# otaviog/align3d

Hardware: AMD Instinct MI355X
Metric: ICP frame-pairs/sec (640x480, 3-lvl, 15 iters) (higher is better)
Workload: dtype f32; 1 GPU; ms3x15 x 64 pairs/GPU, distinct frames, 640x480, 3 lvl x 15 it, HBM-resident (configs[4] shard); pairs_per_gpu=64, global_pairs=64, levels=3, distinct_frames=True, ranks_in_collective=1, collective=none

## Files before the change

### align3d_amd/_abi.py

```python
import ctypes as C
import os
import threading

import numpy as np

A3D_OK = 0
A3D_INVALID_PARAMETER = 1
A3D_MISSING_FIELD = 2
A3D_SOLVE_FAILED = 3
A3D_HIP_ERROR = 4
A3D_NAN_IN_INPUT = 5
A3D_CAST_OVERFLOW = 6

STATUS_NAMES = {
    0: "A3D_OK",
    1: "A3D_INVALID_PARAMETER",
    2: "A3D_MISSING_FIELD",
    3: "A3D_SOLVE_FAILED",
    4: "A3D_HIP_ERROR",
    5: "A3D_NAN_IN_INPUT",
    6: "A3D_CAST_OVERFLOW",
}


# ... 289 lines not shown
    "a3d_pcl_icp_batch_align_device": (_ST, [_P, C.POINTER(PointCloudViewC), C.POINTER(PoseC), C.POINTER(C.c_int32)]),
    "a3d_pcl_icp_batch_results": (_ST, [_P, C.POINTER(PoseC), C.POINTER(C.c_int32)]),
    "a3d_pcl_icp_batch_last_device_ms": (_ST, [_P, C.POINTER(C.c_float)]),
    "a3d_pcl_icp_batch_free": (_ST, [_P]),
    "a3d_bilateral_default_sigmas": (None, [C.POINTER(C.c_double), C.POINTER(C.c_double)]),
    "a3d_bilateral_filter_u16": (
        _ST,
        [_P, _P, C.c_uint64, C.c_uint64, C.c_double, C.c_double, _P, C.POINTER(C.c_uint64)],
    ),
    "a3d_bilateral_filter_u16_device": (_ST, [_P, _P, C.c_uint64, C.c_uint64, C.c_uint64, C.c_double, C.c_double, _P]),
}

DIAG_SIGNATURES = {
    "a3d_image_icp_accumulate_exact": (
        _ST,
        [_P, C.POINTER(IcpParamsC), _P, _P, C.POINTER(PoseC), C.POINTER(GnStateC), C.POINTER(GnStateC)],
    ),
    "a3d_image_icp_accumulate_weighted": (
        _ST,
        [_P, C.POINTER(IcpParamsC), _P, _P, C.POINTER(PoseC), C.POINTER(GnStateC)],
    ),
    "a3d_range_image_download_depth16": (_ST, [_P, _P, C.POINTER(C.c_float), C.POINTER(C.c_int32)]),
    "a3d_backproject_proven": (_ST, [C.c_uint32, C.c_uint32, C.POINTER(C.c_float), C.POINTER(C.c_int32)]),
    "a3d_acos_gate_threshold": (_ST, [C.c_float, C.c_int32, C.POINTER(C.c_float)]),
}

_CSRC = os.path.join(os.path.dirname(os.path.abspath(__file__)), "csrc")
LIB_PATH = os.environ.get("A3D_LIBRARY") or os.path.join(_CSRC, "libalign3d_hip.so")
DIAG_LIB_PATH = os.path.join(_CSRC, "libalign3d_hip_diag.so")
_libs = {}


def load_library(path=None):
    path = os.path.abspath(path or LIB_PATH)
    if path in _libs:
        return _libs[path]
    if not os.path.exists(path):
        raise RuntimeError(
            f"{path} not found: build the HIP extension first "
            "(python -c 'import __graft_entry__ as g; g.build()' or make -C align3d_amd/csrc all)"
        )
    lib = C.CDLL(path)
    for name, (restype, argtypes) in SIGNATURES.items():
        fn = getattr(lib, name)
        fn.restype = restype
        fn.argtypes = argtypes
# ... 32 lines not shown
```

### align3d_amd/csrc/common.hpp

```cpp
#pragma once
#include <hip/hip_runtime.h>

#include <atomic>
#include <memory>
#include <cstdarg>
#include <cstdio>
#include <cstring>
#include <mutex>
#include <string>
#include <utility>
#include <vector>

#include "../../include/align3d_hip.h"
#include "devmath.hpp"

struct a3d_context;

#ifdef A3D_DIAGNOSTICS
#define A3D_DIAG_ENV(name) getenv(name)
#else
#define A3D_DIAG_ENV(name) ((const char*)nullptr)
#endif

namespace a3d {
// ... 78 lines not shown
  hipStream_t copy_stream = nullptr;
  std::vector<hipEvent_t> copy_events;
  unsigned long long grid_capacity = 0;
  struct GridLayoutKey {
    const void* region = nullptr;
    unsigned long long capacity = 0;
    uint32_t cell_bytes = 0, flags_stride = 0, frames = 0, columns = 0;
  } grid_clean;
  uint32_t grid_layout_frames = 0;
  std::vector<std::pair<size_t, uint32_t>> arena_requests;
  struct CachedTable {
    uint32_t key[4];
    void* d;
  };
  std::vector<CachedTable> tables;
  int stream_priority = 0;
  std::mutex stream_mutex;
  std::vector<hipStream_t> side_streams;
  uint64_t build_stats[4] = {0, 0, 0, 0};
  bool build_profiling = false;
  std::vector<hipEvent_t> build_events;
  float last_build_kernel_ms = 0.f;
  uint32_t tiles_per_pair = 0;
  int live_arenas = 0;
  bool zombie = false;
};

namespace a3d {
a3d_status ctx_side_stream(a3d_context* ctx, uint32_t index, hipStream_t* out);
a3d_status ctx_scratch(a3d_context* ctx, int which, size_t bytes, void** out);
a3d_status ctx_block_alloc(a3d_context* ctx, size_t bytes, void** out, size_t* out_bytes);
void ctx_block_release(a3d_context* ctx, void* p, size_t bytes);

struct DeviceArena {
  void* base = nullptr;
  size_t bytes = 0;
  bool slab_slice = false;
  std::atomic<int> refs{0};
  std::mutex fence_mutex;
  std::vector<std::shared_ptr<struct UseFence>> fences;
  std::shared_ptr<struct UseFence> self_fence;
};

struct UseFence {
  std::mutex m;
  hipEvent_t ev = nullptr;
// ... 91 lines not shown
```

### align3d_amd/csrc/devmath.hpp

```cpp
#pragma once
#include <hip/hip_runtime.h>
#include <math.h>

#include <algorithm>
#include <cmath>
#include <stdint.h>

#define A3D_HD __host__ __device__ __forceinline__

namespace a3d {

struct V3 {
  float x, y, z;
};
A3D_HD V3 operator+(V3 a, V3 b) { return {a.x + b.x, a.y + b.y, a.z + b.z}; }
A3D_HD V3 operator-(V3 a, V3 b) { return {a.x - b.x, a.y - b.y, a.z - b.z}; }
A3D_HD V3 operator*(V3 a, float s) { return {a.x * s, a.y * s, a.z * s}; }
A3D_HD V3 operator/(V3 a, float s) { return {a.x / s, a.y / s, a.z / s}; }
A3D_HD float dot(V3 a, V3 b) { return (a.x * b.x + a.y * b.y) + a.z * b.z; }
A3D_HD float norm_squared(V3 a) { return dot(a, a); }
A3D_HD V3 cross(V3 a, V3 b) {
  return {a.y * b.z - a.z * b.y, a.z * b.x - a.x * b.z, a.x * b.y - a.y * b.x};
}

struct Quat {
  float i, j, k, w;
};
struct Pose {
// ... 166 lines not shown

__device__ __forceinline__ V3 backproject_px(uint32_t d, int row, int col, float fx, float fy, float cx, float cy, float scale,
                                             const DivBy dfx, const DivBy dfy, bool focal_ok) {
  V3 p{0.f, 0.f, 0.f};
  if (d > 0) {
    p.z = (float)d * scale;
    const float ax = ((float)col - cx) * p.z, ay = ((float)row - cy) * p.z;
    const bool fast = focal_ok & div_num_ok(ax) & div_num_ok(ay);
    if (__builtin_expect(__builtin_amdgcn_ballot_w64(!fast) != 0ull, 0)) {
      p.x = ax / fx, p.y = ay / fy;
    } else {
      p.x = ax == 0.0f ? ax : div_by(ax, dfx), p.y = ay == 0.0f ? ay : div_by(ay, dfy);
    }
  }
  return p;
}

__device__ __forceinline__ V3 backproject_px_proven(uint32_t d, int row, int col, float cx, float cy, float scale,
                                                    const DivBy dfx, const DivBy dfy) {
  V3 p;
  p.z = (float)d * scale;
  const float ax = ((float)col - cx) * p.z, ay = ((float)row - cy) * p.z;
  p.x = div_by(ax, dfx), p.y = div_by(ay, dfy);
  return p;
}
#endif

inline bool backproject_proven(uint32_t w, uint32_t h, float fx, float fy, float cx, float cy, float scale) {
  if (w == 0 || h == 0 || w > (1u << 24) || h > (1u << 24)) return false;
  if (!(scale >= 1.17549435e-38f)) return false;
  const float zmin = 1.0f * scale, zmax = 65535.0f * scale;
  if (!(zmax <= 3.40282347e38f)) return false;
  auto den_ok = [](float f) { return (std::fabs(f) > 1e-9f) & (std::fabs(f) < 1e9f); };
  auto axis_ok = [&](uint32_t n, float f, float c) {
    if (!den_ok(f) || !std::isfinite(c)) return false;
    float amax = 0.0f, amin = INFINITY;
    bool zero = false;
    const double fl = std::floor(std::min(std::max((double)c, -2.0), (double)n + 1.0));
    const double ks[6] = {0.0, (double)(n - 1), fl - 1.0, fl, fl + 1.0, fl + 2.0};
    for (double kd : ks) {
      const float k = (float)std::min(std::max(kd, 0.0), (double)(n - 1));
      const float a = k - c;
      if (a == 0.0f) {
        if (k != c) return false;
        zero = true;
      } else {
        amax = std::max(amax, std::fabs(a)), amin = std::min(amin, std::fabs(a));
      }
    }
    const float big = amax * zmax;
    if (!(big < 1e9f)) return false;
    if (amin != INFINITY && !(amin * zmin > 1e-20f)) return false;
    return !zero || f > 0.0f;
  };
  return axis_ok(w, fx, cx) && axis_ok(h, fy, cy);
}

#if defined(__HIPCC__)


__device__ __forceinline__ V3 normal_from_neighbours_dev(V3 center, V3 left, V3 right, V3 top, V3 bottom) {
  const float ld = norm_squared(left - center), rd = norm_squared(right - center);
  V3 left_to_right;
  if ((ld < 4.0f * rd) & (4.0f * ld > rd))
    left_to_right = right - left;
  else if (ld < rd)
    left_to_right = center - left;
  else
    left_to_right = right - center;
  const float bd = norm_squared(bottom - center), td = norm_squared(top - center);
  V3 bottom_to_top;
  if ((bd < 4.0f * td) & (4.0f * bd > td))
    bottom_to_top = top - bottom;
  else if (bd < td)
    bottom_to_top = center - bottom;
  else
    bottom_to_top = top - center;
  const V3 n = cross(left_to_right, bottom_to_top);
  const float mag = sqrtf(norm_squared(n));
  V3 out{0.f, 0.f, 0.f};
// ... 42 lines not shown
```

### align3d_amd/csrc/frame.hip

```cpp
#include <cmath>
#include <cstdlib>
#include <memory>

#include "pyramid_ops.hpp"

using namespace a3d;

namespace {

#ifndef A3D_MAX_BATCH
#define A3D_MAX_BATCH 48
#endif
#ifndef A3D_GRID_BUDGET_GB
#define A3D_GRID_BUDGET_GB 4
#endif
constexpr uint32_t MAX_BATCH = A3D_MAX_BATCH;
struct FrameBases {
  char* arena[MAX_BATCH];
};

struct LevelLayout {
  uint32_t w, h;
  size_t points, mask, normals, colors, intensities, imap;
  size_t depth16;
// ... 840 lines not shown
}

#ifdef A3D_DIAGNOSTICS
a3d_status a3d_range_image_download_depth16(a3d_device_image* im, uint16_t* out_depth, float out_backproject[5],
                                            int32_t* out_points_from_depth) {
  A3D_REQUIRE(im && out_depth && out_backproject && out_points_from_depth, A3D_INVALID_PARAMETER, "null argument");
  A3D_REQUIRE(im->depth16, A3D_MISSING_FIELD, "image has no depth plane");
  hipSetDevice(im->ctx->device);
  const size_t n = (size_t)im->width * im->height;
  A3D_HIP_TRY(hipMemcpyAsync(out_depth, im->depth16, n * 2, hipMemcpyDeviceToHost, im->ctx->stream));
  A3D_HIP_TRY(hipStreamSynchronize(im->ctx->stream));
  out_backproject[0] = im->bp_fx, out_backproject[1] = im->bp_fy, out_backproject[2] = im->bp_cx;
  out_backproject[3] = im->bp_cy, out_backproject[4] = im->depth_scale;
  *out_points_from_depth = im->points_from_depth ? 1 : 0;
  return A3D_OK;
}

a3d_status a3d_backproject_proven(uint32_t width, uint32_t height, const float backproject[5], int32_t* out_proven) {
  A3D_REQUIRE(backproject && out_proven, A3D_INVALID_PARAMETER, "null argument");
  const float* k = backproject;
  *out_proven = a3d::backproject_proven(width, height, k[0], k[1], k[2], k[3], k[4]) ? 1 : 0;
  return A3D_OK;
}
#endif

}
```

### align3d_amd/csrc/image_icp.hip

```cpp
#include <cstdlib>
#include <memory>

#include "icp_engine.hpp"

using namespace a3d;

namespace {

struct LevelDesc {
  const float* src_points;
  const uint8_t* src_mask;
  const uint8_t* src_intensities;
  const float* tgt_points;
  const float* tgt_normals;
  const uint8_t* tgt_mask;
  const float* imap;
  uint32_t src_n;
  uint32_t tw, th;
  float fx, fy, cx, cy;
  uint32_t flags;
  uint32_t ppt;
  uint32_t src_w;
  const uint16_t* src_depth;
  const uint16_t* tgt_depth;
  float src_bp[5], tgt_bp[5];
  float src_inv_w;
  uint32_t pad;
};
static_assert(sizeof(LevelDesc) == 160, "LevelDesc layout");

struct Gates {
  float max_distance_sqr;
  float max_color_distance_sqr;
  float dot_reject_max;
};

__device__ __forceinline__ uint32_t f32_as_usize(float x) {
  uint32_t r;
  asm("v_cvt_u32_f32_e32 %0, %1" : "=v"(r) : "v"(x));
  return r;
}
__device__ __forceinline__ int32_t f32_as_i32(float x) {
  int32_t r;
  asm("v_cvt_i32_f32_e32 %0, %1" : "=v"(r) : "v"(x));
  return r;
}

typedef const char __attribute__((address_space(1)))* gptr_c;
template <typename T>
__device__ __forceinline__ T ld(const void* base, uint32_t byte_off) {
  return *(const T __attribute__((address_space(1)))*)((gptr_c)base + byte_off);
}
// ... 9 lines not shown
}


__device__ __forceinline__ uint32_t texel_offset(uint32_t row, uint32_t width, uint32_t col) {
  return (__umul24(row, width) + col) * 4u;
}

__device__ __forceinline__ float bilerp(float v00, float v10, float v01, float v11, float uf, float vf) {
  float u0 = v00 * (1.0f - uf) + v10 * uf;
  float u1 = v01 * (1.0f - uf) + v11 * uf;
  return u0 * (1.0f - vf) + u1 * vf;
}
__device__ __forceinline__ float bilinear_at(const float* imap, uint32_t mw, float u, float v) {
  const uint32_t ui = f32_as_usize(u), vi = f32_as_usize(v);
  const uint32_t o = texel_offset(vi, mw, ui);
  const f32x2 a = ld<f32x2_u>(imap, o), b = ld<f32x2_u>(imap, o + mw * 4u);
  return bilerp(a.x, a.y, b.x, b.y, u - (float)ui, v - (float)vi);
}

struct SrcPx {
  V3 sp;
  uint8_t intensity;
  bool live;
  uint32_t depth, row, col;
};
struct BackProj {
  float fx, fy, cx, cy, scale;
  DivBy dfx, dfy;
};
struct BackProj2 {
  BackProj src, tgt;
};
__device__ __forceinline__ float uniform_f(float x) {
  return __int_as_float(__builtin_amdgcn_readfirstlane(__float_as_int(x)));
}
__device__ __forceinline__ BackProj make_backproj(const float (&k)[5]) {
  BackProj b;
  b.fx = k[0], b.fy = k[1], b.cx = k[2], b.cy = k[3], b.scale = k[4];
  const DivBy dx = div_prepare(b.fx), dy = div_prepare(b.fy);
  b.dfx = DivBy{uniform_f(dx.negz), uniform_f(dx.y)}, b.dfy = DivBy{uniform_f(dy.negz), uniform_f(dy.y)};
  return b;
}
constexpr int D16_TGT = 1, D16_SRC = 2;
#ifndef A3D_ICP_DEPTH16_SRC
#define A3D_ICP_DEPTH16_SRC 1
#endif
constexpr int D16_SIDES = D16_TGT | (A3D_ICP_DEPTH16_SRC ? D16_SRC : 0);
template <bool ZMASK = false, int D16 = 0>
__device__ __forceinline__ SrcPx stage_a(const LevelDesc& d, uint32_t i, bool in_range) {
  const uint32_t ii = in_range ? i : 0u;
  SrcPx s;
  if (D16 & D16_SRC) {
    const uint32_t r = f32_as_usize(((float)ii + 0.5f) * d.src_inv_w);
    s.row = r, s.col = ii - __umul24(r, d.src_w);
    s.depth = ld<uint16_t>(d.src_depth, ii * 2u);
    s.intensity = ld<uint8_t>(d.src_intensities, ii);
    s.live = in_range;
    return s;
  }
  s.sp = ld_v3(d.src_points, ii);
  s.intensity = ld<uint8_t>(d.src_intensities, ii);
  if (ZMASK) {
    s.live = in_range & (s.sp.z != 0.0f);
    return s;
  }
  const uint8_t mask = ld<uint8_t>(d.src_mask, ii);
  s.live = in_range & (mask != 0);
  return s;
}

struct ProjPx {
  V3 p;
  float u, v;
  V3 tp, tn;
  uint8_t tmask;
  bool live;
  uint16_t tdepth;
  uint32_t trow, tcol;
  float t00, t10, t01, t11;
};
template <bool ZMASK = false, int D16 = 0, bool CLASSIC = false>
__device__ __forceinline__ ProjPx stage_b(const LevelDesc& d, const Pose& T, const SrcPx& s, float twf, float thf,
                                          const BackProj2& bp = BackProj2{}) {
  ProjPx o;
  V3 sp = s.sp;
  bool slive = s.live;
  if (D16 & D16_SRC) {
    sp = backproject_px_proven(s.depth, (int)s.row, (int)s.col, bp.src.cx, bp.src.cy, bp.src.scale, bp.src.dfx, bp.src.dfy);
    slive = slive & (s.depth != 0u);
  }
  o.p = transform_vector(T, sp);
  const float z = o.p.z, au = o.p.x * d.fx, av = o.p.y * d.fy;
  const DivBy dz = div_prepare(z);
  float qu = div_by(au, dz), qv = div_by(av, dz);
  if (__builtin_expect(__builtin_amdgcn_ballot_w64(!(div_den_ok(z) & div_num_ok(au) & div_num_ok(av))) != 0ull, 0))
    qu = au / z, qv = av / z;
  o.u = qu + d.cx;
  o.v = qv + d.cy;
  const float ur = o.u + 0.5f, vr = o.v + 0.5f;
  o.live = slive & !((ur <= -1.0f) | (ur >= twf) | (vr <= -1.0f) | (vr >= thf));
  const uint32_t col = (uint32_t)f32_as_i32(ur), row = (uint32_t)f32_as_i32(vr);
  const uint32_t tidx = o.live ? __umul24(row, d.tw) + col : 0u;
  if (D16 & D16_TGT) {
    o.tdepth = ld<uint16_t>(d.tgt_depth, tidx * 2u);
    o.trow = row, o.tcol = col;
    o.tn = ld_v3(d.tgt_normals, tidx);
  } else {
    o.tp = ld_v3(d.tgt_points, tidx);
    o.tn = ld_v3(d.tgt_normals, tidx);
    o.tmask = ZMASK ? (uint8_t)0 : ld<uint8_t>(d.tgt_mask, tidx);
  }
  if (!CLASSIC) {
    const uint32_t mw = d.tw + 2u;
    const uint32_t ui = f32_as_usize(o.u), vi = f32_as_usize(o.v);
    const uint32_t mo = o.live ? texel_offset(vi, mw, ui) : 0u;
    const f32x2 a = ld<f32x2_u>(d.imap, mo), b = ld<f32x2_u>(d.imap, mo + mw * 4u);
    o.t00 = a.x, o.t10 = a.y, o.t01 = b.x, o.t11 = b.y;
  }
  return o;
}

struct MapPx {
  float t00, t10, t01, t11;
  uint32_t ui, vi;
};
template <bool ZMASK = false, int D16 = 0, bool CLASSIC = false>
__device__ __forceinline__ MapPx stage_c(const LevelDesc& d, const Gates& gt, ProjPx& px, uint32_t mw,
                                         const BackProj2& bp = BackProj2{}) {
  bool tvalid;
  if (D16 & D16_TGT) {
    uint32_t wide;
    asm volatile("v_and_b32 %0, 0xffff, %1" : "=v"(wide) : "v"(px.tdepth));
    const uint32_t td = px.live ? wide : 0u;
    px.tp = backproject_px_proven(td, (int)px.trow, (int)px.tcol, bp.tgt.cx, bp.tgt.cy, bp.tgt.scale, bp.tgt.dfx, bp.tgt.dfy);
    tvalid = td != 0u;
  } else {
    tvalid = ZMASK ? px.tp.z != 0.0f : px.tmask == 1;
  }
  const V3 diff = px.tp - px.p;
  const float pn = dot(px.p, px.tn);
  px.live = px.live & tvalid
            & !(norm_squared(diff) > gt.max_distance_sqr)
            & !((pn >= -1.0f) & (pn <= gt.dot_reject_max));
  MapPx m;
  m.ui = f32_as_usize(px.u), m.vi = f32_as_usize(px.v);
  if (!CLASSIC) {
    m.t00 = px.t00, m.t10 = px.t10, m.t01 = px.t01, m.t11 = px.t11;
    return m;
  }
  const uint32_t o = px.live ? texel_offset(m.vi, mw, m.ui) : 0u;
  const f32x2 a = ld<f32x2_u>(d.imap, o), b = ld<f32x2_u>(d.imap, o + mw * 4u);
  m.t00 = a.x, m.t10 = a.y, m.t01 = b.x, m.t11 = b.y;
  return m;
}

struct Terms {
  float Jg[6], rg;
  float Jc[6], rc;
// ... 177 lines not shown
      a[21 + i] = a[21 + i] + m;
    }
    const float rr = r * r;
    a[27] = a[27] + rr;
    a[28] += 1.0f;
  };
  for (int k0 = 0; k0 < PPT; ++k0) {
    const uint32_t i = blockIdx.x * (256u * (uint32_t)PPT) + threadIdx.x + (uint32_t)k0 * 256u;
    const SrcPx s0 = stage_a(d, i, i < d.src_n);
    ProjPx px = stage_b(d, T, s0, twf, thf);
    const MapPx mp = stage_c(d, gt, px, mw);
    if (px.live) {
      const Terms t = stage_d<true>(d, gt, px, mp, s0.intensity, mw);
      step_exact(acc, t.rg, t.Jg);
      if (t.color) step_exact(acc + GN_ACC, t.rc, t.Jc);
    }
  }
  block_reduce_store<GN_PARTIAL, false>(acc, partials + (size_t)blockIdx.x * GN_PARTIAL);
}

#endif

template <bool ZMASK, int D16 = 0>
__device__ __forceinline__ SrcPx pixel_source_at(const LevelDesc& d, uint32_t base, int ppt, int k0) {
  const uint32_t i = base + (uint32_t)k0 * 256u;
  return stage_a<ZMASK, D16>(d, i, (k0 < ppt) && (i < d.src_n));
}
template <bool ZMASK, int D16 = 0, bool CLASSIC = false>
__device__ __forceinline__ void pixel_pass(const LevelDesc& d, const Gates& gt, const Pose& T, uint32_t base, int ppt,
                                           const SrcPx& s0, SrcPx sa, float (&acc)[GN_PARTIAL]) {
  const uint32_t mw = d.tw + 2;
  const float twf = (float)d.tw, thf = (float)d.th;
  BackProj2 bp{};
  if (D16 & D16_SRC) bp.src = make_backproj(d.src_bp);
  if (D16 & D16_TGT) bp.tgt = make_backproj(d.tgt_bp);
  SrcPx sb;
  ProjPx pa = stage_b<ZMASK, D16, CLASSIC>(d, T, s0, twf, thf, bp), pb;
  uint8_t ia = s0.intensity, ib;
  auto step = [&](ProjPx& cur, uint8_t cur_i, ProjPx& nxt, uint8_t& nxt_i, const SrcPx& s_next, SrcPx& s_new, int k0) {
    s_new = pixel_source_at<ZMASK, D16>(d, base, ppt, k0 + 2);
    if constexpr (!CLASSIC) {
      __builtin_amdgcn_sched_barrier(0);
      nxt = stage_b<ZMASK, D16>(d, T, s_next, twf, thf, bp);
      nxt_i = s_next.intensity;
      __builtin_amdgcn_sched_barrier(0);
      const MapPx mp = stage_c<ZMASK, D16>(d, gt, cur, mw, bp);
      if (cur.live) {
        const Terms t = stage_d(d, gt, cur, mp, cur_i, mw);
        gn_step(acc, t.rg, t.Jg);
        if (t.color) gn_step(acc + GN_ACC, t.rc, t.Jc);
      }
      return;
    }
    if (D16) __builtin_amdgcn_sched_barrier(0);
    const MapPx mp = stage_c<ZMASK, D16, true>(d, gt, cur, mw, bp);
    nxt = stage_b<ZMASK, D16, true>(d, T, s_next, twf, thf, bp);
    nxt_i = s_next.intensity;
    if (cur.live) {
      const Terms t = stage_d(d, gt, cur, mp, cur_i, mw);
      gn_step(acc, t.rg, t.Jg);
      if (t.color) gn_step(acc + GN_ACC, t.rc, t.Jc);
    }
  };
#pragma unroll 1
  for (int k0 = 0; k0 < ppt; k0 += 2) {
    step(pa, ia, pb, ib, sa, sb, k0);
    step(pb, ib, pa, ia, sb, sa, k0 + 1);
  }
}

template <bool ZMASK, bool DEPTH16, bool CLASSIC = false>
__global__ void __launch_bounds__(256, 1)
    image_icp_head_kernel(const LevelDesc* __restrict__ descs, const JobState* __restrict__ states_in,
                          JobState* __restrict__ states_out, Gates gt, const float* __restrict__ partials_in,
                          float* __restrict__ partials_out, uint32_t job_stride, HeadArgs head) {
  __shared__ uint32_t s_state[JOB_WORDS];
  const int pair = blockIdx.y;
  const uint32_t tile = blockIdx.x;
  float acc[GN_PARTIAL];
#pragma unroll
  for (int k = 0; k < GN_PARTIAL; ++k) acc[k] = 0.0f;
#if defined(A3D_DIAGNOSTICS) && defined(A3D_TAIL_STAMPS)
  const bool stamping = threadIdx.x == 0 && pair == 0 && tile + 1 == gridDim.x;
  unsigned long long* stamp = g_tail_stamps + 16 + 8 * ((states_out > states_in) ? 1 : 0);
#define A3D_HEAD_STAMP(k) do { if (stamping) stamp[k] = __builtin_amdgcn_s_memrealtime(); } while (0)
#else
#define A3D_HEAD_STAMP(k) do { } while (0)
#endif
  A3D_HEAD_STAMP(0);
  const LevelDesc d = descs[pair];
  const int ppt = (int)d.ppt;
  const uint32_t base = tile * (256u * (uint32_t)ppt) + threadIdx.x;
  constexpr int D16 = DEPTH16 ? D16_SIDES : 0;
  const SrcPx s0 = pixel_source_at<ZMASK, D16>(d, base, ppt, 0), s1 = pixel_source_at<ZMASK, D16>(d, base, ppt, 1);
  A3D_HEAD_STAMP(1);
  head_advance(states_in + pair, tile == 0 ? states_out + pair : nullptr, partials_in + (size_t)pair * job_stride, head,
               pair, s_state, tile == 0);
  A3D_HEAD_STAMP(2);
  if ((int)s_state[15] == A3D_OK) {
    auto uni = [&](int k) { return __uint_as_float(__builtin_amdgcn_readfirstlane(s_state[k])); };
    const Pose T{{uni(0), uni(1), uni(2)}, {uni(3), uni(4), uni(5), uni(6)}};
    pixel_pass<ZMASK, D16, CLASSIC>(d, gt, T, base, ppt, s0, s1, acc);
  }
  A3D_HEAD_STAMP(3);
  block_reduce_store<GN_PARTIAL, false>(acc, partials_out + (size_t)pair * job_stride + (size_t)tile * GN_PARTIAL);
  A3D_HEAD_STAMP(4);
#undef A3D_HEAD_STAMP
}

#ifdef A3D_DIAGNOSTICS
struct PersistLevel {
  uint32_t desc_base;
  uint32_t iterations;
  uint32_t tiles;
  float weight, color_weight;
  Gates gates;
};
constexpr int PERSIST_MAX_LEVELS = 16;
constexpr uint32_t PAIR_CTRL_WORDS = 64;
constexpr uint32_t ROSTER_CLOSED = 0x80000000u;
constexpr unsigned long long ROSTER_WAIT_TICKS = 2000ull, PERSIST_SPIN_BOUND_TICKS = 200'000'000ull;
struct PersistPlan {
  uint32_t n_levels;
  uint32_t seq0;
  uint32_t counter_base;
// ... 430 lines not shown
  unsigned* d_counters = nullptr;
  uint32_t counter_base = 0;
  uint32_t persist_parity = 0;
  uint32_t persist_mask = 0;
  uint32_t persist_resident_blocks = 0;
  bool persist_disabled = false;
  bool persist_used = false;
  std::vector<uint32_t> persist_levels;
  uint32_t last_groups = 1;
  unsigned long long* d_stamps = nullptr;
  Pose* d_poses = nullptr;
  Pose* d_init = nullptr;
  int32_t* d_status = nullptr;
  double* d_readback = nullptr;
  hipEvent_t ev0 = nullptr, ev1 = nullptr;
  std::vector<hipEvent_t> kev;
  std::vector<uint8_t> kev_level;
  float last_level_ms[16] = {0};
  uint32_t last_level_launches[16] = {0};
  bool profile_kernels = false;
  uint32_t resident_blocks = 1024;
  bool zmask = false;
  bool depth16 = false;
  uint32_t n_streams = 1;
  hipStream_t aux_streams[3] = {nullptr, nullptr, nullptr};
  hipEvent_t ev_fork = nullptr, ev_join[3] = {nullptr, nullptr, nullptr};
  float last_total_ms = 0.f, last_kernel_ms = 0.f;
  uint64_t last_kernel_launches = 0;
  const Pose* last_init = nullptr;
  uint32_t last_levels = 0;
  float* last_matrices = nullptr;
  std::shared_ptr<UseFence> fence = std::make_shared<UseFence>();
  std::shared_ptr<UseFence> descs_uploaded = std::make_shared<UseFence>();
#ifdef A3D_DIAGNOSTICS
  unsigned* d_epochs = nullptr;
  bool use_level_kernel = false;
  uint32_t level_mask = 0;
  uint32_t level_resident_blocks = 0;
  bool use_mfma = false, merged_accumulators = false;
  bool head_solve = true;
  bool exact_solve = false;
#endif

  ~a3d_multiscale_batch() {
    fence->retire();
    hipFree(d_block);
    hipFree(d_partials);
    hipFree(d_stamps);
    if (ev0) hipEventDestroy(ev0);
    if (ev1) hipEventDestroy(ev1);
    for (auto e : kev) hipEventDestroy(e);
    for (int i = 0; i < 3; ++i) {
      if (ev_join[i]) hipEventDestroy(ev_join[i]);
    }
    if (ev_fork) hipEventDestroy(ev_fork);
  }
};

namespace {

a3d_status fill_desc(const a3d_device_image* target, const a3d_device_image* source, LevelDesc* d) {
  A3D_REQUIRE(target && source, A3D_INVALID_PARAMETER, "null image handle");
  A3D_REQUIRE(target->has_imap, A3D_MISSING_FIELD, "Please, the target image should have a intensity map.");
  A3D_REQUIRE(target->has_normals, A3D_MISSING_FIELD, "Please, the target image should have normals.");
  A3D_REQUIRE(source->has_intensities, A3D_MISSING_FIELD,
              "Please, the source image should have intensity colors.");
  d->imap = target->imap;
  d->src_points = source->points, d->src_mask = source->mask, d->src_intensities = source->intensities;
  d->tgt_points = target->points, d->tgt_normals = target->normals, d->tgt_mask = target->mask;
  d->src_n = source->width * source->height;
  d->tw = target->width;
  d->th = target->height;
  d->fx = target->fx, d->fy = target->fy, d->cx = target->cx, d->cy = target->cy;
  d->flags = (target->mask_is_z && source->mask_is_z) ? 1u : 0u;
  d->ppt = 2, d->pad = 0;
  d->src_w = source->width;
  d->src_inv_w = 1.0f / (float)std::max(1u, source->width);
  auto proven = [](const a3d_device_image* im) {
    return im->points_from_depth && im->depth16 &&
           backproject_proven(im->width, im->height, im->bp_fx, im->bp_fy, im->bp_cx, im->bp_cy, im->depth_scale);
  };
  const bool from_depth = proven(target) && proven(source);
  if (from_depth) d->flags |= 2u;
  d->src_depth = from_depth ? source->depth16 : nullptr;
  d->tgt_depth = from_depth ? target->depth16 : nullptr;
  const float sbp[5] = {source->bp_fx, source->bp_fy, source->bp_cx, source->bp_cy, source->depth_scale};
  const float tbp[5] = {target->bp_fx, target->bp_fy, target->bp_cx, target->bp_cy, target->depth_scale};
  for (int k = 0; k < 5; ++k) d->src_bp[k] = sbp[k], d->tgt_bp[k] = tbp[k];
  return A3D_OK;
}

Gates make_gates(const a3d_icp_params& p) {
  Gates g;
  g.max_distance_sqr = p.max_distance * p.max_distance;
  g.max_color_distance_sqr = p.max_color_distance * p.max_color_distance;
  g.dot_reject_max = acos_gate_threshold(p.max_normal_angle, false);
  return g;
}

void tiling_for(uint32_t n, uint32_t want, uint32_t group, uint32_t* tiles, uint32_t* ppt) {
  const uint32_t step = std::max(2u, group);
  want = std::max(1u, std::min(want, std::max(1u, (n + 256 * step - 1) / (256 * step))));
  uint32_t p = (n + 256 * want - 1) / (256 * want);
  p = std::max(step, ((p + step - 1) / step) * step);
  *ppt = p;
  *tiles = std::max(1u, (n + 256 * p - 1) / (256 * p));
// ... 105 lines not shown
  const uint32_t P = b->n_pairs;
  const uint32_t job_stride = b->max_tiles * GN_PARTIAL;
  const JobState* st_in = b->d_states + (size_t)(seq & 1u) * P + p0;
  JobState* st_out = b->d_states + (size_t)((seq + 1u) & 1u) * P + p0;
  const float* part_in = b->d_partials + (size_t)((seq + 1u) & 1u) * b->partials_half + (size_t)p0 * job_stride;
  float* part_out = b->d_partials + (size_t)(seq & 1u) * b->partials_half + (size_t)p0 * job_stride;
  const LevelDesc* descs = b->d_descs + (size_t)level * P + p0;
#ifdef A3D_DIAGNOSTICS
  const char* oenv = A3D_DIAG_ENV("A3D_ICP_STEP_ORDER");
  if (oenv && strcmp(oenv, "classic") == 0) {
    if (b->depth16 && level == 0)
      hipLaunchKernelGGL((image_icp_head_kernel<true, true, true>), dim3(b->tiles[level], count), dim3(256), 0, s, descs,
                         st_in, st_out, b->gates[level], part_in, part_out, job_stride, prev);
    else if (b->zmask)
      hipLaunchKernelGGL((image_icp_head_kernel<true, false, true>), dim3(b->tiles[level], count), dim3(256), 0, s, descs,
                         st_in, st_out, b->gates[level], part_in, part_out, job_stride, prev);
    else
      hipLaunchKernelGGL((image_icp_head_kernel<false, false, true>), dim3(b->tiles[level], count), dim3(256), 0, s, descs,
                         st_in, st_out, b->gates[level], part_in, part_out, job_stride, prev);
    A3D_HIP_TRY(hipGetLastError());
    return A3D_OK;
  }
#endif
  if (b->depth16 && level == 0)
    hipLaunchKernelGGL((image_icp_head_kernel<true, true>), dim3(b->tiles[level], count), dim3(256), 0, s, descs, st_in,
                       st_out, b->gates[level], part_in, part_out, job_stride, prev);
  else if (b->zmask)
    hipLaunchKernelGGL((image_icp_head_kernel<true, false>), dim3(b->tiles[level], count), dim3(256), 0, s, descs, st_in,
                       st_out, b->gates[level], part_in, part_out, job_stride, prev);
  else
    hipLaunchKernelGGL((image_icp_head_kernel<false, false>), dim3(b->tiles[level], count), dim3(256), 0, s, descs, st_in,
                       st_out, b->gates[level], part_in, part_out, job_stride, prev);
  A3D_HIP_TRY(hipGetLastError());
  return A3D_OK;
}

a3d_status batch_commit_descs(a3d_multiscale_batch* b) {
  const uint32_t P = b->n_pairs, L = b->n_levels;
  plan_tiling(b);
  size_t max_partials = 1;
  for (uint32_t l = 0; l < L; ++l) max_partials = std::max(max_partials, (size_t)P * b->tiles[l] * GN_PARTIAL);
  b->max_tiles = (uint32_t)(max_partials / ((size_t)P * GN_PARTIAL));
  const char* zenv = A3D_DIAG_ENV("A3D_ICP_ZMASK");
  b->zmask = !(zenv && atoi(zenv) == 0);
  for (const LevelDesc& dsc : b->h_descs) b->zmask = b->zmask && (dsc.flags & 1u);
  const char* denv = A3D_DIAG_ENV("A3D_ICP_DEPTH16");
  b->depth16 = b->zmask && L > 0 && !(denv && atoi(denv) == 0);
  for (uint32_t p = 0; p < P && b->depth16; ++p) {
    const LevelDesc& dsc = b->h_descs[p];
    b->depth16 = (dsc.flags & 2u) && dsc.src_n <= (1u << 22);
  }
  b->partials_half = max_partials;
  if (b->partials_capacity < 2 * max_partials) {
    if (b->d_partials) A3D_HIP_TRY(hipFree(b->d_partials));
    b->d_partials = nullptr;
    b->partials_capacity = 0;
    A3D_HIP_TRY(hipMalloc((void**)&b->d_partials, 2 * max_partials * sizeof(float)));
    b->partials_capacity = 2 * max_partials;
  }
  A3D_HIP_TRY(hipMemcpyAsync(b->d_descs, b->h_descs.data(), b->h_descs.size() * sizeof(LevelDesc),
                             hipMemcpyHostToDevice, b->ctx->stream));
  return A3D_OK;
}

a3d_status batch_create(a3d_context* ctx, const a3d_icp_params* params, uint32_t n_levels, uint32_t n_pairs,
                        std::unique_ptr<a3d_multiscale_batch>* out) {
  auto b = std::make_unique<a3d_multiscale_batch>();
  b->ctx = ctx;
  b->n_pairs = n_pairs;
  b->n_levels = n_levels;
  b->params.assign(params, params + n_levels);
  for (uint32_t l = 0; l < n_levels; ++l) b->gates.push_back(make_gates(params[l]));
  b->tiles.assign(n_levels, 0);
  b->ppt.assign(n_levels, 2);
// ... 774 lines not shown
```

### include/align3d_hip.h

```cpp
#ifndef ALIGN3D_HIP_H
#define ALIGN3D_HIP_H

#include <stddef.h>
#include <stdint.h>

#ifdef __cplusplus
extern "C" {
#endif

#define A3D_ABI_VERSION 1
#define A3D_RENDER_MAX_HALF_WIDTH 8

typedef enum a3d_status {
  A3D_OK = 0,
  A3D_INVALID_PARAMETER = 1,
  A3D_MISSING_FIELD = 2,
  A3D_SOLVE_FAILED = 3,
  A3D_HIP_ERROR = 4,
  A3D_NAN_IN_INPUT = 5,
  A3D_CAST_OVERFLOW = 6
} a3d_status;

typedef struct a3d_icp_params {
  uint64_t max_iterations;
// ... 133 lines not shown
a3d_status a3d_compute_normals(a3d_context* ctx, const float* points, const uint8_t* mask,
                               uint64_t width, uint64_t height, float* out_normals);


a3d_status a3d_image_icp_align(a3d_context* ctx, const a3d_icp_params* params,
                               const a3d_device_image* target, const a3d_device_image* source,
                               const a3d_pose* init_pose, a3d_pose* out_pose);

a3d_status a3d_image_icp_accumulate(a3d_context* ctx, const a3d_icp_params* params,
                                    const a3d_device_image* target, const a3d_device_image* source,
                                    const a3d_pose* pose, a3d_gn_state* out_geom,
                                    a3d_gn_state* out_color);

#ifdef A3D_DIAGNOSTICS
a3d_status a3d_image_icp_accumulate_exact(a3d_context* ctx, const a3d_icp_params* params, const a3d_device_image* target,
                                          const a3d_device_image* source, const a3d_pose* pose,
                                          a3d_gn_state* out_geom, a3d_gn_state* out_color);
a3d_status a3d_image_icp_accumulate_weighted(a3d_context* ctx, const a3d_icp_params* params,
                                             const a3d_device_image* target, const a3d_device_image* source,
                                             const a3d_pose* pose, a3d_gn_state* out_state);
a3d_status a3d_range_image_download_depth16(a3d_device_image* image, uint16_t* out_depth, float out_backproject[5],
                                            int32_t* out_points_from_depth);
a3d_status a3d_backproject_proven(uint32_t width, uint32_t height, const float backproject[5], int32_t* out_proven);
a3d_status a3d_acos_gate_threshold(float thr, int32_t strict, float* out);
#endif

a3d_status a3d_image_icp_align_trace(a3d_context* ctx, const a3d_icp_params* params,
                                     const a3d_device_image* target, const a3d_device_image* source,
                                     const a3d_pose* init_pose, a3d_pose* out_pose, float* out_trace);

a3d_status a3d_selftest_transform(a3d_context* ctx, const float* updates6, const a3d_pose* poses, const float* points3,
                                  uint64_t n, a3d_pose* out_composed, float* out_points3, float* out_normals3);
a3d_status a3d_selftest_division(a3d_context* ctx, const float* numerators, const float* denominators,
                                 uint64_t n, uint64_t* out_mismatches);


a3d_status a3d_multiscale_new(a3d_context* ctx, const a3d_icp_params* params, uint64_t n_params,
                              const a3d_device_image* const* target_pyramid, uint64_t n_levels,
                              a3d_multiscale** out);
a3d_status a3d_multiscale_align(a3d_multiscale* ms, const a3d_device_image* const* source_pyramid,
                                uint64_t n_source_levels, a3d_pose* out_pose);
a3d_status a3d_multiscale_align_host(a3d_multiscale* ms, const a3d_range_image_view* source_pyramid,
                                     uint64_t n_source_levels, a3d_pose* out_pose);
a3d_status a3d_multiscale_free(a3d_multiscale* ms);

a3d_status a3d_multiscale_batch_new(a3d_context* ctx, const a3d_icp_params* params,
// ... 176 lines not shown
```

Before: 25540 frame-pairs/s.

## Use host-verified short reciprocal division and incremental row/col in depth16 ICP head

On the host, each focal length is checked by an exhaustive sweep over all float mantissas to prove that a two-FMA reciprocal division is bit-exact. When every focal length passes, level 0 runs a specialized head kernel that uses the precomputed reciprocals instead of the full div_by sequence. The kernel also derives source row/col by incremental float stride advance instead of a per-pixel multiply-divide, and converts target depth with an SDWA cvt. The cost is a one-time 8M-iteration host sweep per distinct focal length, cached per context, plus a larger LevelDesc.

Measured after the change: 25890 frame-pairs/s, median of 6. About the same (+1.4%).

```diff
diff --git a/align3d_amd/_abi.py b/align3d_amd/_abi.py
--- a/align3d_amd/_abi.py
+++ b/align3d_amd/_abi.py
@@ -335,6 +335,7 @@
     ),
     "a3d_range_image_download_depth16": (_ST, [_P, _P, C.POINTER(C.c_float), C.POINTER(C.c_int32)]),
     "a3d_backproject_proven": (_ST, [C.c_uint32, C.c_uint32, C.POINTER(C.c_float), C.POINTER(C.c_int32)]),
+    "a3d_backproject_short_division_proven": (_ST, [C.c_uint32, C.c_uint32, C.POINTER(C.c_float), C.POINTER(C.c_int32)]),
     "a3d_acos_gate_threshold": (_ST, [C.c_float, C.c_int32, C.POINTER(C.c_float)]),
 }
 
diff --git a/align3d_amd/csrc/common.hpp b/align3d_amd/csrc/common.hpp
--- a/align3d_amd/csrc/common.hpp
+++ b/align3d_amd/csrc/common.hpp
@@ -124,6 +124,8 @@
   std::vector<hipEvent_t> build_events;
   float last_build_kernel_ms = 0.f;
   uint32_t tiles_per_pair = 0;
+  std::mutex short_div_mutex;
+  std::vector<std::pair<uint32_t, bool>> short_div_verdicts;
   int live_arenas = 0;
   bool zombie = false;
 };
diff --git a/align3d_amd/csrc/devmath.hpp b/align3d_amd/csrc/devmath.hpp
--- a/align3d_amd/csrc/devmath.hpp
+++ b/align3d_amd/csrc/devmath.hpp
@@ -4,6 +4,7 @@
 
 #include <algorithm>
 #include <cmath>
+#include <cstring>
 #include <stdint.h>
 
 #define A3D_HD __host__ __device__ __forceinline__
@@ -216,6 +217,19 @@
   p.z = (float)d * scale;
   const float ax = ((float)col - cx) * p.z, ay = ((float)row - cy) * p.z;
   p.x = div_by(ax, dfx), p.y = div_by(ay, dfy);
+  return p;
+}
+__device__ __forceinline__ float div_short(float a, const DivBy d) {
+  const float q = a * d.y;
+  return __builtin_fmaf(__builtin_fmaf(d.negz, q, a), d.y, q);
+}
+template <bool SHORT>
+__device__ __forceinline__ V3 backproject_px_proven_f(float d, float row, float col, float cx, float cy, float scale,
+                                                      const DivBy dfx, const DivBy dfy) {
+  V3 p;
+  p.z = d * scale;
+  const float ax = (col - cx) * p.z, ay = (row - cy) * p.z;
+  p.x = SHORT ? div_short(ax, dfx) : div_by(ax, dfx), p.y = SHORT ? div_short(ay, dfy) : div_by(ay, dfy);
   return p;
 }
 #endif
@@ -250,6 +264,38 @@
   return axis_ok(w, fx, cx) && axis_ok(h, fy, cy);
 }
 
+#if defined(__x86_64__) && !defined(__HIP_DEVICE_COMPILE__)
+#define A3D_HOST_FMA 1
+#define A3D_HOST_FMA_TARGET __attribute__((target("fma")))
+#else
+#define A3D_HOST_FMA 0
+#define A3D_HOST_FMA_TARGET
+#endif
+template <bool HW>
+__attribute__((always_inline)) inline bool short_division_sweep(float f, float y) {
+  const float nf = -f;
+  uint32_t bad = 0;
+  for (uint32_t m = 0; m < (1u << 23); ++m) {
+    const uint32_t bits = 0x3f800000u | m;
+    float a;
+    memcpy(&a, &bits, 4);
+    const float q = a * y;
+    const float r = HW ? __builtin_fmaf(nf, q, a) : std::fmaf(nf, q, a);
+    const float q1 = HW ? __builtin_fmaf(r, y, q) : std::fmaf(r, y, q);
+    bad |= (uint32_t)(q1 != a / f);
+  }
+  return bad == 0;
+}
+A3D_HOST_FMA_TARGET inline bool short_division_sweep_fma(float f, float y) { return short_division_sweep<true>(f, y); }
+inline bool short_division_proven(float f) {
+  if (!((std::fabs(f) > 1e-9f) & (std::fabs(f) < 1e9f))) return false;
+  const float y = 1.0f / f;
+#if A3D_HOST_FMA
+  if (__builtin_cpu_supports("fma")) return short_division_sweep_fma(f, y);
+#endif
+  return short_division_sweep<false>(f, y);
+}
+
 #if defined(__HIPCC__)
 
 
diff --git a/align3d_amd/csrc/frame.hip b/align3d_amd/csrc/frame.hip
--- a/align3d_amd/csrc/frame.hip
+++ b/align3d_amd/csrc/frame.hip
@@ -886,6 +886,17 @@
   *out_proven = a3d::backproject_proven(width, height, k[0], k[1], k[2], k[3], k[4]) ? 1 : 0;
   return A3D_OK;
 }
-#endif
-
-}
+
+a3d_status a3d_backproject_short_division_proven(uint32_t width, uint32_t height, const float backproject[5],
+                                                 int32_t* out_proven) {
+  A3D_REQUIRE(backproject && out_proven, A3D_INVALID_PARAMETER, "null argument");
+  const float* k = backproject;
+  *out_proven = (a3d::backproject_proven(width, height, k[0], k[1], k[2], k[3], k[4]) && a3d::short_division_proven(k[0]) &&
+                 a3d::short_division_proven(k[1]))
+                    ? 1
+                    : 0;
+  return A3D_OK;
+}
+#endif
+
+}
diff --git a/align3d_amd/csrc/image_icp.hip b/align3d_amd/csrc/image_icp.hip
--- a/align3d_amd/csrc/image_icp.hip
+++ b/align3d_amd/csrc/image_icp.hip
@@ -26,8 +26,9 @@
   float src_bp[5], tgt_bp[5];
   float src_inv_w;
   uint32_t pad;
+  float src_rcp_f[2], tgt_rcp_f[2];
 };
-static_assert(sizeof(LevelDesc) == 160, "LevelDesc layout");
+static_assert(sizeof(LevelDesc) == 176, "LevelDesc layout");
 
 struct Gates {
   float max_distance_sqr;
@@ -83,8 +84,23 @@
   V3 sp;
   uint8_t intensity;
   bool live;
-  uint32_t depth, row, col;
+  uint32_t depth;
+  float row, col;
 };
+struct SrcStride {
+  float q, q1, r, w;
+};
+__device__ __forceinline__ SrcStride make_src_stride(uint32_t w) {
+  w = w ? w : 1u;
+  const uint32_t q = 256u / w;
+  return {(float)q, (float)(q + 1u), (float)(256u - q * w), (float)w};
+}
+__device__ __forceinline__ void src_advance(const SrcStride& st, float row, float col, float* nrow, float* ncol) {
+  const float c = col + st.r;
+  const bool wrap = c >= st.w;
+  *ncol = wrap ? c - st.w : c;
+  *nrow = row + (wrap ? st.q1 : st.q);
+}
 struct BackProj {
   float fx, fy, cx, cy, scale;
   DivBy dfx, dfy;
@@ -95,9 +111,14 @@
 __device__ __forceinline__ float uniform_f(float x) {
   return __int_as_float(__builtin_amdgcn_readfirstlane(__float_as_int(x)));
 }
-__device__ __forceinline__ BackProj make_backproj(const float (&k)[5]) {
+template <bool SHORT = false>
+__device__ __forceinline__ BackProj make_backproj(const float (&k)[5], const float (&rcp_f)[2]) {
   BackProj b;
   b.fx = k[0], b.fy = k[1], b.cx = k[2], b.cy = k[3], b.scale = k[4];
+  if (SHORT) {
+    b.dfx = DivBy{-b.fx, rcp_f[0]}, b.dfy = DivBy{-b.fy, rcp_f[1]};
+    return b;
+  }
   const DivBy dx = div_prepare(b.fx), dy = div_prepare(b.fy);
   b.dfx = DivBy{uniform_f(dx.negz), uniform_f(dx.y)}, b.dfy = DivBy{uniform_f(dy.negz), uniform_f(dy.y)};
   return b;
@@ -108,12 +129,17 @@
 #endif
 constexpr int D16_SIDES = D16_TGT | (A3D_ICP_DEPTH16_SRC ? D16_SRC : 0);
 template <bool ZMASK = false, int D16 = 0>
-__device__ __forceinline__ SrcPx stage_a(const LevelDesc& d, uint32_t i, bool in_range) {
+__device__ __forceinline__ SrcPx stage_a(const LevelDesc& d, uint32_t i, bool in_range, const SrcPx* prev = nullptr,
+                                         const SrcStride* stride = nullptr) {
   const uint32_t ii = in_range ? i : 0u;
   SrcPx s;
   if (D16 & D16_SRC) {
-    const uint32_t r = f32_as_usize(((float)ii + 0.5f) * d.src_inv_w);
-    s.row = r, s.col = ii - __umul24(r, d.src_w);
+    if (prev) {
+      src_advance(*stride, prev->row, prev->col, &s.row, &s.col);
+    } else {
+      const uint32_t r = f32_as_usize(((float)i + 0.5f) * d.src_inv_w);
+      s.row = (float)r, s.col = (float)(i - __umul24(r, d.src_w));
+    }
     s.depth = ld<uint16_t>(d.src_depth, ii * 2u);
     s.intensity = ld<uint8_t>(d.src_intensities, ii);
     s.live = in_range;
@@ -136,18 +162,18 @@
   V3 tp, tn;
   uint8_t tmask;
   bool live;
-  uint16_t tdepth;
+  _Float16 tdepth;
   uint32_t trow, tcol;
   float t00, t10, t01, t11;
 };
-template <bool ZMASK = false, int D16 = 0, bool CLASSIC = false>
+template <bool ZMASK = false, int D16 = 0, bool CLASSIC = false, bool SHORT = false>
 __device__ __forceinline__ ProjPx stage_b(const LevelDesc& d, const Pose& T, const SrcPx& s, float twf, float thf,
                                           const BackProj2& bp = BackProj2{}) {
   ProjPx o;
   V3 sp = s.sp;
   bool slive = s.live;
   if (D16 & D16_SRC) {
-    sp = backproject_px_proven(s.depth, (int)s.row, (int)s.col, bp.src.cx, bp.src.cy, bp.src.scale, bp.src.dfx, bp.src.dfy);
+    sp = backproject_px_proven_f<SHORT>((float)s.depth, s.row, s.col, bp.src.cx, bp.src.cy, bp.src.scale, bp.src.dfx, bp.src.dfy);
     slive = slive & (s.depth != 0u);
   }
   o.p = transform_vector(T, sp);
@@ -163,7 +189,7 @@
   const uint32_t col = (uint32_t)f32_as_i32(ur), row = (uint32_t)f32_as_i32(vr);
   const uint32_t tidx = o.live ? __umul24(row, d.tw) + col : 0u;
   if (D16 & D16_TGT) {
-    o.tdepth = ld<uint16_t>(d.tgt_depth, tidx * 2u);
+    o.tdepth = ld<_Float16>(d.tgt_depth, tidx * 2u);
     o.trow = row, o.tcol = col;
     o.tn = ld_v3(d.tgt_normals, tidx);
   } else {
@@ -185,16 +211,17 @@
   float t00, t10, t01, t11;
   uint32_t ui, vi;
 };
-template <bool ZMASK = false, int D16 = 0, bool CLASSIC = false>
+template <bool ZMASK = false, int D16 = 0, bool CLASSIC = false, bool SHORT = false>
 __device__ __forceinline__ MapPx stage_c(const LevelDesc& d, const Gates& gt, ProjPx& px, uint32_t mw,
                                          const BackProj2& bp = BackProj2{}) {
   bool tvalid;
   if (D16 & D16_TGT) {
-    uint32_t wide;
-    asm volatile("v_and_b32 %0, 0xffff, %1" : "=v"(wide) : "v"(px.tdepth));
-    const uint32_t td = px.live ? wide : 0u;
-    px.tp = backproject_px_proven(td, (int)px.trow, (int)px.tcol, bp.tgt.cx, bp.tgt.cy, bp.tgt.scale, bp.tgt.dfx, bp.tgt.dfy);
-    tvalid = td != 0u;
+    float wide;
+    asm volatile("v_cvt_f32_u32_sdwa %0, %1 dst_sel:DWORD dst_unused:UNUSED_PAD src0_sel:WORD_0" : "=v"(wide) : "v"(px.tdepth));
+    const float td = px.live ? wide : 0.0f;
+    px.tp = backproject_px_proven_f<SHORT>(td, (float)(int)px.trow, (float)(int)px.tcol, bp.tgt.cx, bp.tgt.cy,
+                                           bp.tgt.scale, bp.tgt.dfx, bp.tgt.dfy);
+    tvalid = td != 0.0f;
   } else {
     tvalid = ZMASK ? px.tp.z != 0.0f : px.tmask == 1;
   }
@@ -418,29 +445,32 @@
 #endif
 
 template <bool ZMASK, int D16 = 0>
-__device__ __forceinline__ SrcPx pixel_source_at(const LevelDesc& d, uint32_t base, int ppt, int k0) {
+__device__ __forceinline__ SrcPx pixel_source_at(const LevelDesc& d, uint32_t base, int ppt, int k0,
+                                                 const SrcPx* prev = nullptr, const SrcStride* stride = nullptr) {
   const uint32_t i = base + (uint32_t)k0 * 256u;
-  return stage_a<ZMASK, D16>(d, i, (k0 < ppt) && (i < d.src_n));
-}
-template <bool ZMASK, int D16 = 0, bool CLASSIC = false>
+  return stage_a<ZMASK, D16>(d, i, (k0 < ppt) && (i < d.src_n), prev, stride);
+}
+template <bool ZMASK, int D16 = 0, bool CLASSIC = false, bool SHORT = false>
 __device__ __forceinline__ void pixel_pass(const LevelDesc& d, const Gates& gt, const Pose& T, uint32_t base, int ppt,
                                            const SrcPx& s0, SrcPx sa, float (&acc)[GN_PARTIAL]) {
   const uint32_t mw = d.tw + 2;
   const float twf = (float)d.tw, thf = (float)d.th;
   BackProj2 bp{};
-  if (D16 & D16_SRC) bp.src = make_backproj(d.src_bp);
-  if (D16 & D16_TGT) bp.tgt = make_backproj(d.tgt_bp);
+  if (D16 & D16_SRC) bp.src = make_backproj<SHORT>(d.src_bp, d.src_rcp_f);
+  if (D16 & D16_TGT) bp.tgt = make_backproj<SHORT>(d.tgt_bp, d.tgt_rcp_f);
+  SrcStride stride{};
+  if (D16 & D16_SRC) stride = make_src_stride(d.src_w);
   SrcPx sb;
-  ProjPx pa = stage_b<ZMASK, D16, CLASSIC>(d, T, s0, twf, thf, bp), pb;
+  ProjPx pa = stage_b<ZMASK, D16, CLASSIC, SHORT>(d, T, s0, twf, thf, bp), pb;
   uint8_t ia = s0.intensity, ib;
   auto step = [&](ProjPx& cur, uint8_t cur_i, ProjPx& nxt, uint8_t& nxt_i, const SrcPx& s_next, SrcPx& s_new, int k0) {
-    s_new = pixel_source_at<ZMASK, D16>(d, base, ppt, k0 + 2);
+    s_new = pixel_source_at<ZMASK, D16>(d, base, ppt, k0 + 2, &s_next, &stride);
     if constexpr (!CLASSIC) {
       __builtin_amdgcn_sched_barrier(0);
-      nxt = stage_b<ZMASK, D16>(d, T, s_next, twf, thf, bp);
+      nxt = stage_b<ZMASK, D16, false, SHORT>(d, T, s_next, twf, thf, bp);
       nxt_i = s_next.intensity;
       __builtin_amdgcn_sched_barrier(0);
-      const MapPx mp = stage_c<ZMASK, D16>(d, gt, cur, mw, bp);
+      const MapPx mp = stage_c<ZMASK, D16, false, SHORT>(d, gt, cur, mw, bp);
       if (cur.live) {
         const Terms t = stage_d(d, gt, cur, mp, cur_i, mw);
         gn_step(acc, t.rg, t.Jg);
@@ -449,8 +479,8 @@
       return;
     }
     if (D16) __builtin_amdgcn_sched_barrier(0);
-    const MapPx mp = stage_c<ZMASK, D16, true>(d, gt, cur, mw, bp);
-    nxt = stage_b<ZMASK, D16, true>(d, T, s_next, twf, thf, bp);
+    const MapPx mp = stage_c<ZMASK, D16, true, SHORT>(d, gt, cur, mw, bp);
+    nxt = stage_b<ZMASK, D16, true, SHORT>(d, T, s_next, twf, thf, bp);
     nxt_i = s_next.intensity;
     if (cur.live) {
       const Terms t = stage_d(d, gt, cur, mp, cur_i, mw);
@@ -465,7 +495,7 @@
   }
 }
 
-template <bool ZMASK, bool DEPTH16, bool CLASSIC = false>
+template <bool ZMASK, bool DEPTH16, bool CLASSIC = false, bool SHORT = false>
 __global__ void __launch_bounds__(256, 1)
     image_icp_head_kernel(const LevelDesc* __restrict__ descs, const JobState* __restrict__ states_in,
                           JobState* __restrict__ states_out, Gates gt, const float* __restrict__ partials_in,
@@ -488,7 +518,9 @@
   const int ppt = (int)d.ppt;
   const uint32_t base = tile * (256u * (uint32_t)ppt) + threadIdx.x;
   constexpr int D16 = DEPTH16 ? D16_SIDES : 0;
-  const SrcPx s0 = pixel_source_at<ZMASK, D16>(d, base, ppt, 0), s1 = pixel_source_at<ZMASK, D16>(d, base, ppt, 1);
+  SrcStride stride{};
+  if (D16 & D16_SRC) stride = make_src_stride(d.src_w);
+  const SrcPx s0 = pixel_source_at<ZMASK, D16>(d, base, ppt, 0), s1 = pixel_source_at<ZMASK, D16>(d, base, ppt, 1, &s0, &stride);
   A3D_HEAD_STAMP(1);
   head_advance(states_in + pair, tile == 0 ? states_out + pair : nullptr, partials_in + (size_t)pair * job_stride, head,
                pair, s_state, tile == 0);
@@ -496,7 +528,7 @@
   if ((int)s_state[15] == A3D_OK) {
     auto uni = [&](int k) { return __uint_as_float(__builtin_amdgcn_readfirstlane(s_state[k])); };
     const Pose T{{uni(0), uni(1), uni(2)}, {uni(3), uni(4), uni(5), uni(6)}};
-    pixel_pass<ZMASK, D16, CLASSIC>(d, gt, T, base, ppt, s0, s1, acc);
+    pixel_pass<ZMASK, D16, CLASSIC, SHORT>(d, gt, T, base, ppt, s0, s1, acc);
   }
   A3D_HEAD_STAMP(3);
   block_reduce_store<GN_PARTIAL, false>(acc, partials_out + (size_t)pair * job_stride + (size_t)tile * GN_PARTIAL);
@@ -973,6 +1005,7 @@
   uint32_t resident_blocks = 1024;
   bool zmask = false;
   bool depth16 = false;
+  bool short_div = false;
   uint32_t n_streams = 1;
   hipStream_t aux_streams[3] = {nullptr, nullptr, nullptr};
   hipEvent_t ev_fork = nullptr, ev_join[3] = {nullptr, nullptr, nullptr};
@@ -1009,6 +1042,17 @@
 };
 
 namespace {
+
+bool short_division_cached(a3d_context* ctx, float f) {
+  uint32_t key;
+  memcpy(&key, &f, 4);
+  std::lock_guard<std::mutex> lock(ctx->short_div_mutex);
+  for (const auto& kv : ctx->short_div_verdicts)
+    if (kv.first == key) return kv.second;
+  const bool ok = short_division_proven(f);
+  ctx->short_div_verdicts.emplace_back(key, ok);
+  return ok;
+}
 
 a3d_status fill_desc(const a3d_device_image* target, const a3d_device_image* source, LevelDesc* d) {
   A3D_REQUIRE(target && source, A3D_INVALID_PARAMETER, "null image handle");
@@ -1033,6 +1077,11 @@
   };
   const bool from_depth = proven(target) && proven(source);
   if (from_depth) d->flags |= 2u;
+  if (from_depth && short_division_cached(target->ctx, target->bp_fx) && short_division_cached(target->ctx, target->bp_fy) &&
+      short_division_cached(target->ctx, source->bp_fx) && short_division_cached(target->ctx, source->bp_fy))
+    d->flags |= 4u;
+  d->src_rcp_f[0] = 1.0f / source->bp_fx, d->src_rcp_f[1] = 1.0f / source->bp_fy;
+  d->tgt_rcp_f[0] = 1.0f / target->bp_fx, d->tgt_rcp_f[1] = 1.0f / target->bp_fy;
   d->src_depth = from_depth ? source->depth16 : nullptr;
   d->tgt_depth = from_depth ? target->depth16 : nullptr;
   const float sbp[5] = {source->bp_fx, source->bp_fy, source->bp_cx, source->bp_cy, source->depth_scale};
@@ -1184,7 +1233,10 @@
     return A3D_OK;
   }
 #endif
-  if (b->depth16 && level == 0)
+  if (b->depth16 && level == 0 && b->short_div)
+    hipLaunchKernelGGL((image_icp_head_kernel<true, true, false, true>), dim3(b->tiles[level], count), dim3(256), 0, s, descs,
+                       st_in, st_out, b->gates[level], part_in, part_out, job_stride, prev);
+  else if (b->depth16 && level == 0)
     hipLaunchKernelGGL((image_icp_head_kernel<true, true>), dim3(b->tiles[level], count), dim3(256), 0, s, descs, st_in,
                        st_out, b->gates[level], part_in, part_out, job_stride, prev);
   else if (b->zmask)
@@ -1212,6 +1264,9 @@
     const LevelDesc& dsc = b->h_descs[p];
     b->depth16 = (dsc.flags & 2u) && dsc.src_n <= (1u << 22);
   }
+  const char* senv = A3D_DIAG_ENV("A3D_ICP_SHORT_DIV");
+  b->short_div = b->depth16 && !(senv && atoi(senv) == 0);
+  for (uint32_t p = 0; p < P && b->short_div; ++p) b->short_div = (b->h_descs[p].flags & 4u) != 0;
   b->partials_half = max_partials;
   if (b->partials_capacity < 2 * max_partials) {
     if (b->d_partials) A3D_HIP_TRY(hipFree(b->d_partials));
diff --git a/include/align3d_hip.h b/include/align3d_hip.h
--- a/include/align3d_hip.h
+++ b/include/align3d_hip.h
@@ -179,6 +179,8 @@
 a3d_status a3d_range_image_download_depth16(a3d_device_image* image, uint16_t* out_depth, float out_backproject[5],
                                             int32_t* out_points_from_depth);
 a3d_status a3d_backproject_proven(uint32_t width, uint32_t height, const float backproject[5], int32_t* out_proven);
+a3d_status a3d_backproject_short_division_proven(uint32_t width, uint32_t height, const float backproject[5],
+                                                 int32_t* out_proven);
 a3d_status a3d_acos_gate_threshold(float thr, int32_t strict, float* out);
 #endif
 
```
